# OpenDriveLab/OccNet

Measured on NVIDIA H100. Metric: samples/s (6-cam->200x200x16 voxel), higher is better.
Workload: dtype bf16

## Files before the change

### include/occ_b200.h

```cpp
#ifndef OCC_B200_H_
#define OCC_B200_H_

#include <stdint.h>

#ifdef __cplusplus
extern "C" {
#endif

const char* occb200_last_error(void);
const char* occb200_version(void);

int occb200_ms_deform_attn_forward(const float* value, const int64_t* spatial_shapes,
                                   const int64_t* level_start_index, const float* sampling_loc,
                                   const float* attn_weight, int B, int Nv, int M, int C, int Nq, int L, int P,
                                   int im2col_step, float* out, void* stream);

int occb200_ms_deform_attn_backward(const float* value, const int64_t* spatial_shapes, const int64_t* level_start_index,
                                    const float* sampling_loc, const float* attn_weight, const float* grad_output, int B,
                                    int Nv, int M, int C, int Nq, int L, int P, int im2col_step, float* grad_value,
                                    float* grad_sampling_loc, float* grad_attn_weight, void* stream);

typedef struct occb200_engine occb200_engine;
typedef struct occb200_backbone occb200_backbone;

typedef struct occb200_config {
    int bev_h, bev_w;
    int embed_dims, num_heads;
    int num_layers;
    int num_cams;
    int num_levels;
    int level_h[4], level_w[4];
    int num_points_in_pillar;
    int sca_points, tsa_points;
    int ffn_dim;
    int pillar_h, out_dim;
    int num_classes;
    float pc_range[6];
    int precision;
    int use_tensor_cores;
    int use_cams_embeds;
    int rotate_center[2];
} occb200_config;

int occb200_engine_create(const occb200_config* cfg, occb200_engine** out);
void occb200_engine_destroy(occb200_engine* e);

int occb200_engine_load_param(occb200_engine* e, const char* key, const float* data, int64_t numel);
int occb200_engine_finalize(occb200_engine* e);

int occb200_engine_set_cameras(occb200_engine* e, const float* cam_mat, const float* zs, int img_h, int img_w);

int occb200_engine_set_prev_rotation(occb200_engine* e, const int32_t* map_host);

int occb200_engine_set_input_dtype(occb200_engine* e, int feats_bf16);
int occb200_engine_attach_backbone(occb200_engine* e, occb200_backbone* bb);

int occb200_engine_forward(occb200_engine* e, const float* const* feats, const float* prev_bev, float* bev_embed,
                           float* occ_logits, float* flow, uint8_t* occ_cls_u8, int64_t* occ_cls_i64, void* stream);

int occb200_engine_forward_host(occb200_engine* e, const float* const* feats_host, int64_t* occ_cls_i64_host,
                                float* flow_host, void* stream);

int occb200_engine_submit_host(occb200_engine* e, int slot, const float* const* feats_host, int64_t* occ_cls_i64_host,
                               float* flow_host, void* stream);
int occb200_engine_wait_host(occb200_engine* e, int slot);

int occb200_engine_enable_taps(occb200_engine* e, int enable);
int occb200_engine_copy_tap(occb200_engine* e, int which, int layer, float* dst_dev, void* stream);

int occb200_engine_project_pillars(occb200_engine* e, float* ref_cam, uint8_t* mask, void* stream);
int occb200_engine_launches_per_frame(const occb200_engine* e);
int occb200_engine_profile(occb200_engine* e, int enable);
int occb200_engine_profile_read(occb200_engine* e, float* ms_per_category, int* launches_per_category, int n);

int occb200_render_forward(const float* sigma, const float* origin, const float* points, const float* tindex,
                           int N, int T, int Z, int Y, int X, int64_t M, float* pred_dist, float* gt_dist,
                           float* coord_index, void* stream);

int occb200_ray_metric_accumulate(const uint8_t* sem_pred, const float* flow_pred, const uint8_t* sem_gt,
                                  const float* flow_gt, const void* origins, int origin_is_f64, int T,
                                  const float* rays, int M, double* counters, float* pcd_pred, float* pcd_gt,
                                  void* stream);

int occb200_linear_f32(const float* A, const float* W, const float* bias, const float* residual, float* C, int M,
                       int N, int K, int act, void* stream);
int occb200_layernorm_f32(const float* x, const float* gamma, const float* beta, float* y, int rows, int C,
                          void* stream);
int occb200_gemm_bf16_tc(const void* A_bf16, const void* W_bf16, const float* bias, float* C, int M, int N, int K,
                         void* stream);

occb200_backbone* occb200_backbone_create(int num_images, int img_h, int img_w, int precision, int use_tensor_cores);
void occb200_backbone_destroy(occb200_backbone* e);
int occb200_backbone_load_param(occb200_backbone* e, const char* key, const float* data, int64_t numel);
int occb200_backbone_finalize(occb200_backbone* e);
int occb200_backbone_level_shape(const occb200_backbone* e, int level, int* h, int* w);
int occb200_backbone_forward(occb200_backbone* e, const float* img, float* out0, float* out1, float* out2, float* out3,
                             void* stream);
int occb200_backbone_forward_nhwc_bf16(occb200_backbone* e, const float* img, void* out0, void* out1, void* out2, void* out3,
                                       void* stream);
int occb200_backbone_set_frame_format(occb200_backbone* e, int src_h, int src_w, const float mean[3], const float std[3],
                                      int to_rgb);
int occb200_backbone_forward_frames(occb200_backbone* e, const uint8_t* frames, void* out0, void* out1, void* out2,
                                    void* out3, int out_layout, void* stream);

#ifdef __cplusplus
}
#endif
#endif
```

### occnet_b200/_lib.py

```python
import ctypes
import os

_HERE = os.path.dirname(os.path.abspath(__file__))
LIB_PATH = os.path.join(_HERE, 'lib', 'libocc_b200.so')

c_f32p = ctypes.c_void_p
_vp = ctypes.c_void_p
_i = ctypes.c_int
_i64 = ctypes.c_int64


class OccConfig(ctypes.Structure):
    _fields_ = [('bev_h', _i), ('bev_w', _i), ('embed_dims', _i), ('num_heads', _i), ('num_layers', _i),
                ('num_cams', _i), ('num_levels', _i), ('level_h', _i * 4), ('level_w', _i * 4),
                ('num_points_in_pillar', _i), ('sca_points', _i), ('tsa_points', _i), ('ffn_dim', _i),
                ('pillar_h', _i), ('out_dim', _i), ('num_classes', _i), ('pc_range', ctypes.c_float * 6),
                ('precision', _i), ('use_tensor_cores', _i), ('use_cams_embeds', _i),
                ('rotate_center', _i * 2)]


SIGNATURES = {
    'occb200_last_error': (ctypes.c_char_p, []),
    'occb200_version': (ctypes.c_char_p, []),
    'occb200_ms_deform_attn_forward': (_i, [_vp, _vp, _vp, _vp, _vp, _i, _i, _i, _i, _i, _i, _i, _i, _vp, _vp]),
    'occb200_ms_deform_attn_backward': (_i, [_vp, _vp, _vp, _vp, _vp, _vp, _i, _i, _i, _i, _i, _i, _i, _i, _vp, _vp, _vp, _vp]),
    'occb200_engine_create': (_i, [ctypes.POINTER(OccConfig), ctypes.POINTER(_vp)]),
    'occb200_engine_destroy': (None, [_vp]),
    'occb200_engine_load_param': (_i, [_vp, ctypes.c_char_p, _vp, _i64]),
    'occb200_engine_finalize': (_i, [_vp]),
    'occb200_engine_set_cameras': (_i, [_vp, _vp, _vp, _i, _i]),
    'occb200_engine_set_input_dtype': (_i, [_vp, _i]),
    'occb200_engine_attach_backbone': (_i, [_vp, _vp]),
    'occb200_engine_set_prev_rotation': (_i, [_vp, _vp]),
    'occb200_engine_forward': (_i, [_vp, ctypes.POINTER(_vp), _vp, _vp, _vp, _vp, _vp, _vp, _vp]),
    'occb200_engine_forward_host': (_i, [_vp, ctypes.POINTER(_vp), _vp, _vp, _vp]),
    'occb200_engine_submit_host': (_i, [_vp, _i, ctypes.POINTER(_vp), _vp, _vp, _vp]),
    'occb200_engine_wait_host': (_i, [_vp, _i]),
    'occb200_engine_enable_taps': (_i, [_vp, _i]),
    'occb200_engine_copy_tap': (_i, [_vp, _i, _i, _vp, _vp]),
    'occb200_engine_project_pillars': (_i, [_vp, _vp, _vp, _vp]),
    'occb200_engine_launches_per_frame': (_i, [_vp]),
    'occb200_engine_profile': (_i, [_vp, _i]),
    'occb200_engine_profile_read': (_i, [_vp, _vp, _vp, _i]),
    'occb200_render_forward': (_i, [_vp, _vp, _vp, _vp, _i, _i, _i, _i, _i, _i64, _vp, _vp, _vp, _vp]),
    'occb200_ray_metric_accumulate': (_i, [_vp, _vp, _vp, _vp, _vp, _i, _i, _vp, _i, _vp, _vp, _vp, _vp]),
    'occb200_linear_f32': (_i, [_vp, _vp, _vp, _vp, _vp, _i, _i, _i, _i, _vp]),
    'occb200_layernorm_f32': (_i, [_vp, _vp, _vp, _vp, _i, _i, _vp]),
    'occb200_gemm_bf16_tc': (_i, [_vp, _vp, _vp, _vp, _i, _i, _i, _vp]),
    'occb200_backbone_create': (_vp, [_i, _i, _i, _i, _i]),
    'occb200_backbone_destroy': (None, [_vp]),
    'occb200_backbone_load_param': (_i, [_vp, ctypes.c_char_p, _vp, ctypes.c_int64]),
    'occb200_backbone_finalize': (_i, [_vp]),
    'occb200_backbone_level_shape': (_i, [_vp, _i, ctypes.POINTER(_i), ctypes.POINTER(_i)]),
    'occb200_backbone_forward': (_i, [_vp, _vp, _vp, _vp, _vp, _vp, _vp]),
    'occb200_backbone_forward_nhwc_bf16': (_i, [_vp, _vp, _vp, _vp, _vp, _vp, _vp]),
    'occb200_backbone_set_frame_format': (_i, [_vp, _i, _i, _vp, _vp, _i]),
    'occb200_backbone_forward_frames': (_i, [_vp, _vp, _vp, _vp, _vp, _vp, _i, _vp]),
}

_lib = None


def load():
    global _lib
    if _lib is None:
        if not os.path.exists(LIB_PATH):
            raise RuntimeError(f'{LIB_PATH} is missing: run `python -m occnet_b200.build` '
                               '(libocc_b200 has no CPU / PyTorch fallback)')
        lib = ctypes.CDLL(LIB_PATH)
        for name, (res, args) in SIGNATURES.items():
            fn = getattr(lib, name)
            fn.restype = res
            fn.argtypes = args
        _lib = lib
    return _lib


class OccB200Error(RuntimeError):
    pass


def check(rc):
    if rc != 0:
        raise OccB200Error(f'libocc_b200 error {rc}: {load().occb200_last_error().decode()}')


def ptr(t):
    if t is None:
        return None
    if hasattr(t, 'data_ptr'):
        return ctypes.c_void_p(t.data_ptr())
    return ctypes.c_void_p(t.ctypes.data)


def stream_ptr():
    import torch
    return ctypes.c_void_p(torch.cuda.current_stream().cuda_stream)
```

### occnet_b200/csrc/engine.cu

```cuda
#include <cuda_runtime.h>

#include <algorithm>
#include <cmath>
#include <cstring>
#include <map>
#include <string>
#include <vector>

#include "../../include/occ_b200.h"
#include "common.cuh"
#include "conv3d_tc.cuh"
#include "gemm_tc.cuh"
#include "kernels.cuh"

namespace occ {

static thread_local std::string g_last_error;
void set_last_error(const std::string& msg) { g_last_error = msg; }

namespace {

struct DevBuf {
    void* p = nullptr;
    size_t bytes = 0;
// ... 1075 lines not shown
    OCC_CHECK(e && (slot == 0 || slot == 1), "bad arguments");
    occb200_engine::Slot& s = e->slots[slot];
    if (!s.busy) return 0;
    OCC_CUDA(cudaEventSynchronize(s.d2h_done));
    s.busy = false;
    return 0;
}

int occb200_engine_set_prev_rotation(occb200_engine* e, const int32_t* map_host)
{
    OCC_CHECK(e, "null engine");
    if (map_host == nullptr) { e->rot_set = false; return 0; }
    for (int q = 0; q < e->Nq; ++q) OCC_CHECK(map_host[q] >= -1 && map_host[q] < e->Nq, "rotation map entry out of range");
    if (e->rot_map.bytes != (size_t)e->Nq * 4 && e->rot_map.alloc((size_t)e->Nq * 4)) return 2;
    OCC_CUDA(cudaMemcpy(e->rot_map.p, map_host, (size_t)e->Nq * 4, cudaMemcpyHostToDevice));
    e->rot_set = true;
    return 0;
}

int occb200_engine_set_input_dtype(occb200_engine* e, int feats_bf16)
{
    OCC_CHECK(e && feats_bf16 >= 0 && feats_bf16 <= 3,
              "input dtype must be 0 (fp32 NCHW), 1 (bf16 NCHW), 2 (bf16 NHWC) or 3 (uint8 camera frames)");
    e->feats_bf16 = feats_bf16;
    return 0;
}

int occb200_engine_attach_backbone(occb200_engine* e, occb200_backbone* bb)
{
    OCC_CHECK(e, "null engine");
    if (bb && check_backbone(e, bb)) return 1;
    if (e->bb_free_recorded) OCC_CUDA(cudaEventSynchronize(e->bb_free));
    e->bb = bb;
    e->bb_free_recorded = false;
    return 0;
}

int occb200_engine_enable_taps(occb200_engine* e, int enable)
{
    OCC_CHECK(e && e->finalized, "engine not finalized");
    e->taps = enable != 0;
    if (e->taps) {
        const size_t n = (size_t)e->cfg.num_layers * e->Nq * 256 * 4;
        if (e->tap_layer.alloc(n) || e->tap_tsa.alloc(n) || e->tap_sca.alloc(n)) return 2;
    }
    return 0;
}

int occb200_engine_copy_tap(occb200_engine* e, int which, int layer, float* dst, void* stream)
{
    OCC_CHECK(e && dst, "null pointer");
    cudaStream_t st = (cudaStream_t)stream;
    const size_t n = (size_t)e->Nq * 256;
    if (which >= 0 && which <= 2) {
        OCC_CHECK(e->taps && layer >= 0 && layer < e->cfg.num_layers, "taps not enabled or bad layer");
        const DevBuf& b = which == 0 ? e->tap_layer : (which == 1 ? e->tap_tsa : e->tap_sca);
        OCC_CUDA(cudaMemcpyAsync(dst, b.as<float>() + layer * n, n * 4, cudaMemcpyDeviceToDevice, st));
        return 0;
    }
    if (which == 3) {
        const size_t nv = (size_t)e->cfg.bev_w * e->cfg.bev_h * e->cfg.pillar_h * e->cfg.out_dim;
        if (e->cfg.precision == 0) {
            OCC_CUDA(cudaMemcpyAsync(dst, e->vox2.p, nv * 4, cudaMemcpyDeviceToDevice, st));
            return 0;
        }
        return launch_bf16_to_f32(e->vox2.as<bf16>(), dst, (int64_t)nv, st);
    }
    if (which == 4) {
        const size_t nt = (size_t)e->cfg.num_cams * e->Nv * 256;
        if (e->cfg.precision == 0) {
            OCC_CUDA(cudaMemcpyAsync(dst, e->tokens.p, nt * 4, cudaMemcpyDeviceToDevice, st));
            return 0;
        }
        return launch_bf16_to_f32(e->tokens.as<bf16>(), dst, (int64_t)nt, st);
    }
    set_last_error("unknown tap");
    return 1;
}

int occb200_engine_project_pillars(occb200_engine* e, float* ref_cam, uint8_t* mask, void* stream)
{
    OCC_CHECK(e && ref_cam && mask && e->cameras_set, "null pointer / cameras not set");
    return launch_project_pillars(e->sp, ref_cam, mask, (cudaStream_t)stream);
}

int occb200_engine_launches_per_frame(const occb200_engine* e) { return e ? e->launches : 0; }

int occb200_engine_profile(occb200_engine* e, int enable)
{
    OCC_CHECK(e, "null engine");
    e->profiling = enable != 0;
    e->prof_events.clear();
    e->event_used = 0;
    return 0;
}

int occb200_engine_profile_read(occb200_engine* e, float* ms_per_category, int* launches_per_category, int n)
{
    OCC_CHECK(e && ms_per_category && launches_per_category && n >= CAT_COUNT, "bad arguments");
    OCC_CUDA(cudaDeviceSynchronize());
    for (int i = 0; i < n; ++i) { ms_per_category[i] = 0.f; launches_per_category[i] = 0; }
    for (auto& pe : e->prof_events) {
        float ms = 0.f;
        OCC_CUDA(cudaEventElapsedTime(&ms, pe.second.first, pe.second.second));
        ms_per_category[pe.first] += ms;
        launches_per_category[pe.first] += 1;
    }
    e->prof_events.clear();
    e->event_used = 0;
    return 0;
}

int occb200_render_forward(const float* sigma, const float* origin, const float* points, const float* tindex, int N,
                           int T, int Z, int Y, int X, int64_t M, float* pred_dist, float* gt_dist, float* coord_index,
                           void* stream)
{
    OCC_CHECK(sigma && origin && points && tindex && pred_dist && gt_dist && coord_index, "null pointer");
    return launch_render_forward(sigma, origin, points, tindex, N, T, Z, Y, X, M, pred_dist, gt_dist, coord_index,
                                 (cudaStream_t)stream);
}

int occb200_ray_metric_accumulate(const uint8_t* sem_pred, const float* flow_pred, const uint8_t* sem_gt,
                                  const float* flow_gt, const void* origins, int origin_is_f64, int T, const float* rays,
                                  int M, double* counters, float* pcd_pred, float* pcd_gt, void* stream)
{
    if (T == 0 || M == 0) return 0;
    OCC_CHECK(sem_pred && flow_pred && sem_gt && flow_gt && origins && rays && counters, "null pointer");
    return launch_ray_metric(sem_pred, flow_pred, sem_gt, flow_gt, origins, origin_is_f64, T, rays, M, counters,
                             pcd_pred, pcd_gt, (cudaStream_t)stream);
}

int occb200_linear_f32(const float* A, const float* W, const float* bias, const float* residual, float* C, int M, int N,
                       int K, int act, void* stream)
{
    OCC_CHECK(A && W && C, "null pointer");
    return gemm_simt<float, float>(A, K, nullptr, 0, K, W, bias, residual, N, C, N, M, N, K, act, (cudaStream_t)stream);
}

int occb200_layernorm_f32(const float* x, const float* gamma, const float* beta, float* y, int rows, int C, void* stream)
{
    OCC_CHECK(x && gamma && beta && y, "null pointer");
    return launch_layernorm<float>(x, gamma, beta, nullptr, rows, C, y, (float*)nullptr, (float*)nullptr,
                                   (cudaStream_t)stream);
}

int occb200_gemm_bf16_tc(const void* A, const void* W, const float* bias, float* C, int M, int N, int K, void* stream)
{
    OCC_CHECK(A && W && C, "null pointer");
    OCC_CHECK(gemm_tc_supported(M, N, K, K), "shape not supported by the tensor-core GEMM");
    return gemm_tc<float>(reinterpret_cast<const bf16*>(A), nullptr, 0, reinterpret_cast<const bf16*>(W), bias, nullptr,
                          C, M, N, K, ACT_NONE, (cudaStream_t)stream);
}

}
```

### occnet_b200/csrc/gemm_tc.cu

```cuda
#include <cstdlib>
#include <map>
#include <mutex>
#include <tuple>
#include <type_traits>

#include "gemm_tc.cuh"
#include "tc_common.cuh"

namespace occ {

PFN_encodeTiled get_encode_tiled()
{
    static PFN_encodeTiled fn = nullptr;
    static std::once_flag once;
    std::call_once(once, [] {
        void* p = nullptr;
        cudaDriverEntryPointQueryResult q;
        if (cudaGetDriverEntryPoint("cuTensorMapEncodeTiled", &p, cudaEnableDefault, &q) == cudaSuccess &&
            q == cudaDriverEntryPointSuccess)
            fn = reinterpret_cast<PFN_encodeTiled>(p);
    });
    return fn;
}

int make_tensor_map_bf16(CUtensorMap* map, const void* base, int rank, const uint64_t* dims, const uint64_t* strides_bytes,
                         const uint32_t* box, int swizzle_bytes)
{
    PFN_encodeTiled enc = get_encode_tiled();
    OCC_CHECK(enc != nullptr, "cuTensorMapEncodeTiled is not available from the driver");
    cuuint64_t gdim[5], gstr[5];
    cuuint32_t bdim[5], estr[5];
    for (int i = 0; i < rank; ++i) { gdim[i] = dims[i]; bdim[i] = box[i]; estr[i] = 1; }
    for (int i = 0; i + 1 < rank; ++i) gstr[i] = strides_bytes[i];
    const CUtensorMapSwizzle sw = swizzle_bytes == 128 ? CU_TENSOR_MAP_SWIZZLE_128B
                                : swizzle_bytes == 64 ? CU_TENSOR_MAP_SWIZZLE_64B
                                : swizzle_bytes == 32 ? CU_TENSOR_MAP_SWIZZLE_32B : CU_TENSOR_MAP_SWIZZLE_NONE;
    const CUresult r = enc(map, CU_TENSOR_MAP_DATA_TYPE_BFLOAT16, (cuuint32_t)rank, const_cast<void*>(base), gdim, gstr,
                           bdim, estr, CU_TENSOR_MAP_INTERLEAVE_NONE, sw, CU_TENSOR_MAP_L2_PROMOTION_L2_128B,
                           CU_TENSOR_MAP_FLOAT_OOB_FILL_NONE);
    OCC_CHECK(r == CUDA_SUCCESS, "cuTensorMapEncodeTiled failed with code " + std::to_string((int)r));
    return 0;
}

int cached_map_2d(const void* base, uint64_t inner, uint64_t rows, uint32_t box_inner, uint32_t box_rows, CUtensorMap* out,
                  uint64_t ld = 0);

namespace {

constexpr int BLOCK_M = 128, BLOCK_K = 64, A_TILE_BYTES = BLOCK_M * BLOCK_K * 2;
constexpr int NUM_THREADS = 384;
constexpr int SMEM_TAIL = 3072 + 256;
constexpr int SMEM_MAX = 232448 - 1024;
constexpr int MAX_STAGES = 6;

struct LnArgs {
    const float* gamma; const float* beta; const float* pos;
    float* y_f32; bf16* y_bf16; bf16* y_pos_bf16;
};

constexpr int MAX_PROBS = 3;
struct GemmProb {
    CUtensorMap tmA, tmA2, tmW;
    const float* bias; const float* residual; void* C;
    const float* res_t32;
    long long ldc, nblk_stride;
    int head_major;
    int M, N, BN, nk, nk1, act, w_resident, stages;
    int out_half;
    int cta_begin, cta_count;
};
struct GemmProbs { GemmProb p[MAX_PROBS]; int n; };

template <typename TC, bool LN>
__global__ void __launch_bounds__(NUM_THREADS, 1)
gemm_tc_kernel(const __grid_constant__ GemmProbs probs, LnArgs ln)
{
    int pi = 0;
    while (pi + 1 < probs.n && (int)blockIdx.x >= probs.p[pi + 1].cta_begin) ++pi;
    const GemmProb& P = probs.p[pi];
    const float* __restrict__ residual = P.residual;
    const float* __restrict__ res_t32 = P.res_t32;
    const int M = P.M, N = P.N, BN = P.BN, nk = P.nk, nk1 = P.nk1, act = P.act;
    const int w_resident = P.w_resident, stages = P.stages;
    const bool out_half = std::is_same<TC, __half>::value || P.out_half != 0;
    const int bid = (int)blockIdx.x - P.cta_begin, nctas = P.cta_count;
    asm volatile("griddepcontrol.launch_dependents;" ::: "memory");
    extern __shared__ uint8_t smem_raw[];
    const uint32_t smem_base = (tc::smem_u32(smem_raw) + 1023u) & ~1023u;
    const uint32_t w_tile_bytes = BN * BLOCK_K * 2;
    const uint32_t w_region = w_resident ? nk * w_tile_bytes : 0;
    const uint32_t stage_bytes = A_TILE_BYTES + (w_resident ? 0 : w_tile_bytes);
    const uint32_t ring_base = smem_base + w_region;
    const uint32_t cvec_base = ring_base + stages * stage_bytes;
    const uint32_t bar_base = cvec_base + 3072;
    auto full_bar = [&](int s) { return bar_base + s * 8; };
    auto empty_bar = [&](int s) { return bar_base + (MAX_STAGES + s) * 8; };
    auto w_bar = [&](int kb) { return bar_base + (2 * MAX_STAGES + (kb < 7 ? kb : 7)) * 8; };
    float* const cvec = reinterpret_cast<float*>(smem_raw + (cvec_base - tc::smem_u32(smem_raw)));

    const int warp = threadIdx.x >> 5, lane = threadIdx.x & 31;
    const int n_tiles = N / BN;
    const int n_blk = bid % n_tiles;
    const int grp = bid / n_tiles, ngrp = nctas / n_tiles;
    const int nb32 = (M + 31) >> 5;
    const int row_begin = (int)(((long long)nb32 * grp) / ngrp) << 5;
    const int row_end = min(M, (int)(((long long)nb32 * (grp + 1)) / ngrp) << 5);

    if (warp == 8 && lane == 0) {
        tc::tma_prefetch_desc(&P.tmA); tc::tma_prefetch_desc(&P.tmA2); tc::tma_prefetch_desc(&P.tmW);
        for (int s = 0; s < stages; ++s) { tc::mbar_init(full_bar(s), 1); tc::mbar_init(empty_bar(s), 2); }
        for (int kb = 0; kb < 8; ++kb) tc::mbar_init(w_bar(kb), 1);
        tc::mbar_fence_init();
    }
    if (threadIdx.x < BN) {
        const int t = threadIdx.x;
        cvec[t] = P.bias ? __ldg(P.bias + n_blk * BN + t) : 0.f;
        if constexpr (LN) { cvec[256 + t] = __ldg(ln.gamma + t); cvec[512 + t] = __ldg(ln.beta + t); }
    }
    __syncthreads();

    if (warp >= 8) {
        tc::setmaxnreg_dec<40>();
        if (warp == 8 && lane == 0) {
            if (w_resident) {
                for (int kb = 0; kb < nk && kb < 8; ++kb)
                    tc::mbar_arrive_expect_tx(w_bar(kb), kb < 7 ? w_tile_bytes : (nk - 7) * w_tile_bytes);
                for (int kb = 0; kb < nk; ++kb)
                    tc::tma_load_2d(smem_base + kb * w_tile_bytes, &P.tmW, w_bar(kb), kb * BLOCK_K, n_blk * BN);
            }
            int s = 0; uint32_t ph = 0;
            asm volatile("griddepcontrol.wait;" ::: "memory");
            for (int m_row = row_begin; m_row < row_end; m_row += BLOCK_M) {
                for (int kb = 0; kb < nk; ++kb) {
                    tc::mbar_wait(empty_bar(s), ph ^ 1);
                    tc::mbar_arrive_expect_tx(full_bar(s), stage_bytes);
                    const uint32_t a_dst = ring_base + s * stage_bytes;
                    if (kb < nk1) tc::tma_load_2d(a_dst, &P.tmA, full_bar(s), kb * BLOCK_K, m_row);
                    else          tc::tma_load_2d(a_dst, &P.tmA2, full_bar(s), (kb - nk1) * BLOCK_K, m_row);
                    if (!w_resident)
                        tc::tma_load_2d(a_dst + A_TILE_BYTES, &P.tmW, full_bar(s), kb * BLOCK_K, n_blk * BN);
                    if (++s == stages) { s = 0; ph ^= 1; }
                }
            }
        }
        return;
    }

    tc::setmaxnreg_inc<232>();
    const int wg = warp >> 2, wl = warp & 3;
    const int nsubs = BN >> 6;
    const int quad_col = 2 * (lane & 3);
    int s = 0; uint32_t ph = 0;
    int tcount = 0;
    asm volatile("griddepcontrol.wait;" ::: "memory");
    for (int m_row = row_begin; m_row < row_end; m_row += BLOCK_M, ++tcount) {
        float acc[4][32];
        for (int kb = 0; kb < nk; ++kb) {
            if (w_resident && tcount == 0) tc::mbar_wait(w_bar(kb), 0);
            tc::mbar_wait(full_bar(s), ph);
            const uint32_t a_addr = ring_base + s * stage_bytes + wg * (64 * 128);
            const uint32_t b_addr = w_resident ? smem_base + kb * w_tile_bytes : ring_base + s * stage_bytes + A_TILE_BYTES;
            switch (nsubs) {
            case 4: tc::wgmma_kblock<4>(acc, a_addr, b_addr, kb == 0); break;
            case 3: tc::wgmma_kblock<3>(acc, a_addr, b_addr, kb == 0); break;
            case 2: tc::wgmma_kblock<2>(acc, a_addr, b_addr, kb == 0); break;
            default: tc::wgmma_kblock<1>(acc, a_addr, b_addr, kb == 0); break;
            }
            if ((threadIdx.x & 127) == 0) tc::mbar_arrive(empty_bar(s));
            if (++s == stages) { s = 0; ph ^= 1; }
        }
        const int r0 = m_row + wg * 64 + wl * 16 + (lane >> 2);
        if constexpr (LN) {
            tc::ln_epilogue(acc, r0, row_end, quad_col, cvec, residual, ln.pos, ln.y_f32, ln.y_bf16, ln.y_pos_bf16);
        } else {
            const bool has_t32 = res_t32 != nullptr, has_res = residual != nullptr, relu = act == ACT_RELU;
            const float* __restrict__ qsrc = has_t32 ? res_t32 : residual;
            const int q_blk = has_t32 ? 1024 : 32, q_j = has_t32 ? 256 : 8;
            const size_t o_blk = P.head_major ? (size_t)M * 32 : 32;
#pragma unroll
            for (int h = 0; h < 2; ++h) {
                const int row = r0 + 8 * h;
                if (row >= row_end) continue;
                const float* const qrow =
                    qsrc + (has_t32 ? ((((size_t)(row >> 5) * (N >> 5) + n_blk * (BN >> 5)) * 256 + (quad_col >> 2) * 32 + (row & 31)) << 2) +
                                          (quad_col & 3)
                                    : (size_t)row * N + n_blk * BN + quad_col);
                float2 q[4][8];
                if (qsrc) {
#pragma unroll
                    for (int ns = 0; ns < 4; ++ns) {
                        if (ns >= nsubs) break;
#pragma unroll
                        for (int j = 0; j < 8; ++j)
                            q[ns][j] = __ldg(reinterpret_cast<const float2*>(qrow + (2 * ns + j / 4) * q_blk + (j & 3) * q_j));
                    }
                }
                TC* const orow = reinterpret_cast<TC*>(P.C) +
                                 (P.head_major ? ((size_t)n_blk * (BN >> 5) * M + row) * 32 + quad_col
                                               : (size_t)n_blk * P.nblk_stride + (size_t)row * P.ldc + quad_col);
#pragma unroll
                for (int ns = 0; ns < 4; ++ns) {
                    if (ns >= nsubs) break;
#pragma unroll
                    for (int j = 0; j < 8; ++j) {
                        const int cl = ns * 64 + 8 * j + quad_col;
                        float x0 = acc[ns][4 * j + 2 * h] + cvec[cl], x1 = acc[ns][4 * j + 2 * h + 1] + cvec[cl + 1];
                        if (has_t32) { x0 += q[ns][j].x; x1 += q[ns][j].y; }
                        if (relu) { x0 = fmaxf(x0, 0.f); x1 = fmaxf(x1, 0.f); }
                        if (has_res) { x0 += q[ns][j].x; x1 += q[ns][j].y; }
                        TC* const o = orow + (2 * ns + j / 4) * o_blk + 8 * (j & 3);
                        if constexpr (sizeof(TC) == 4)
                            *reinterpret_cast<float2*>(o) = make_float2(x0, x1);
                        else
                            *reinterpret_cast<uint32_t*>(o) = tc::pack_16(x0, x1, out_half);
                    }
                }
            }
        }
    }
}

struct Plan { int BN, resident, stages, smem; };

Plan make_plan(int N, int K, bool ln)
{
    const int SMEM_LIMIT = SMEM_MAX - SMEM_TAIL;
    Plan p{0, 0, 0, 0};
    const int cands[] = {256, 192, 128, 64};
    if (ln) {
        p.BN = 256;
    } else {
        for (int bn : cands) {
            if (N % bn != 0 || bn > N) continue;
            if ((long)bn * K * 2 <= 131072) { p.BN = bn; break; }
        }
        if (K > 512 && p.BN != 0 && p.BN < 128) p.BN = 0;
        if (p.BN == 0) {
            for (int bn : cands) if (N % bn == 0 && bn <= N) { p.BN = bn; break; }
        }
    }
    if (p.BN == 0) return p;
    const int w_bytes = p.BN * K * 2;
    p.resident = w_bytes <= 131072;
    const int stage = A_TILE_BYTES + (p.resident ? 0 : p.BN * BLOCK_K * 2);
    const int avail = SMEM_LIMIT - (p.resident ? w_bytes : 0);
    p.stages = avail / stage;
    if (p.stages > MAX_STAGES) p.stages = MAX_STAGES;
    p.smem = 1024 + (p.resident ? w_bytes : 0) + p.stages * stage + SMEM_TAIL;
    return p;
}

struct MapKey {
    const void* p; uint64_t d0, d1, ld; uint32_t b0, b1;
    bool operator<(const MapKey& o) const { return std::tie(p, d0, d1, ld, b0, b1) < std::tie(o.p, o.d0, o.d1, o.ld, o.b0, o.b1); }
};

}

int cached_map_2d(const void* base, uint64_t inner, uint64_t rows, uint32_t box_inner, uint32_t box_rows, CUtensorMap* out,
                  uint64_t ld)
{
    static std::map<MapKey, CUtensorMap> cache;
    static std::mutex mu;
    std::lock_guard<std::mutex> g(mu);
    if (ld == 0) ld = inner;
    const MapKey k{base, inner, rows, ld, box_inner, box_rows};
    auto it = cache.find(k);
    if (it == cache.end()) {
        CUtensorMap m;
        const uint64_t dims[2] = {inner, rows}, strides[1] = {ld * 2};
        const uint32_t box[2] = {box_inner, box_rows};
        if (make_tensor_map_bf16(&m, base, 2, dims, strides, box, 128)) return 1;
        if (cache.size() > 4096) cache.clear();
        it = cache.emplace(k, m).first;
    }
    *out = it->second;
    return 0;
}

namespace {

template <typename TC, bool LN>
int build_prob(GemmProb& P, int& smem, const bf16* A, const bf16* A2, int K1, const bf16* W, const float* bias, const float* residual,
               TC* C, int M, int N, int K, int act, bool blocked_out, int lda, int lda2, bool head_major, int ctas, int cta_begin)
{
    if (A2 == nullptr) K1 = K;
    const Plan p = make_plan(N, K, LN);
    OCC_CHECK(p.BN > 0 && p.stages >= 2 && K % 64 == 0 && K1 % 64 == 0 && M > 0, "gemm_tc: unsupported shape");
    if (cached_map_2d(A, (uint64_t)K1, (uint64_t)M, BLOCK_K, BLOCK_M, &P.tmA, (uint64_t)lda)) return 1;
    if (A2) { if (cached_map_2d(A2, (uint64_t)(K - K1), (uint64_t)M, BLOCK_K, BLOCK_M, &P.tmA2, (uint64_t)lda2)) return 1; }
    else P.tmA2 = P.tmA;
    if (cached_map_2d(W, (uint64_t)K, (uint64_t)N, BLOCK_K, (uint32_t)p.BN, &P.tmW)) return 1;
    if (ctas <= 0) ctas = sm_count_current_device();
    const int m_tiles = (M + BLOCK_M - 1) / BLOCK_M, n_tiles = N / p.BN;
    int per_n = ctas / n_tiles;
    if (per_n > m_tiles) per_n = m_tiles;
    OCC_CHECK(per_n >= 1, "gemm_tc: fewer CTAs than n-blocks");
    P.bias = bias; P.residual = residual; P.C = C; P.res_t32 = nullptr;
    P.ldc = blocked_out ? (long long)p.BN : (long long)N;
    P.nblk_stride = blocked_out ? (long long)M * p.BN : (long long)p.BN;
    P.head_major = head_major ? 1 : 0;
    P.M = M; P.N = N; P.BN = p.BN; P.nk = K / BLOCK_K; P.nk1 = K1 / BLOCK_K; P.act = act;
    P.w_resident = p.resident; P.stages = p.stages;
    P.out_half = std::is_same<TC, __half>::value ? 1 : 0;
    P.cta_begin = cta_begin; P.cta_count = per_n * n_tiles;
    smem = p.smem;
    return 0;
}

template <typename TC, bool LN>
int launch_probs(const GemmProbs& probs, int smem, LnArgs ln, cudaStream_t stream)
{
    OCC_CUDA(cudaFuncSetAttribute(gemm_tc_kernel<TC, LN>, cudaFuncAttributeMaxDynamicSharedMemorySize, 232448));
    const GemmProb& last = probs.p[probs.n - 1];
    const int grid = last.cta_begin + last.cta_count;
    cudaLaunchConfig_t cfg = {};
    cfg.gridDim = dim3(grid); cfg.blockDim = dim3(NUM_THREADS); cfg.dynamicSmemBytes = smem; cfg.stream = stream;
    cudaLaunchAttribute attr[1];
    attr[0].id = cudaLaunchAttributeProgrammaticStreamSerialization;
    attr[0].val.programmaticStreamSerializationAllowed = 1;
    cfg.attrs = attr; cfg.numAttrs = 1;
    OCC_CUDA(cudaLaunchKernelEx(&cfg, gemm_tc_kernel<TC, LN>, probs, ln));
    OCC_CUDA(cudaGetLastError());
    return 0;
}

template <typename TC, bool LN>
int launch(const bf16* A, const bf16* A2, int K1, const bf16* W, const float* bias, const float* residual, TC* C,
           LnArgs ln, int M, int N, int K, int act, cudaStream_t stream, bool blocked_out = false, int lda = 0, int lda2 = 0,
           bool head_major = false)
{
    GemmProbs probs;
    probs.n = 1;
    int smem = 0;
    if (build_prob<TC, LN>(probs.p[0], smem, A, A2, K1, W, bias, residual, C, M, N, K, act, blocked_out, lda, lda2, head_major, 0, 0))
        return 1;
    return launch_probs<TC, LN>(probs, smem, ln, stream);
}

}

bool gemm_tc_supported(int M, int N, int K, int K1)
{
    const Plan p = make_plan(N, K, false);
    return M > 0 && p.BN >= 64 && p.BN % 64 == 0 && p.stages >= 2 && K % 64 == 0 && K1 % 64 == 0 && K1 > 0 && K1 <= K;
}

template <typename TC>
int gemm_tc(const bf16* A, const bf16* A2, int K1, const bf16* W, const float* bias, const float* residual, TC* C,
            int M, int N, int K, int act, cudaStream_t stream)
{
    return launch<TC, false>(A, A2, K1, W, bias, residual, C, LnArgs{}, M, N, K, act, stream);
}

int gemm_tc_heads256(const bf16* A, const bf16* W, const float* bias, bf16* C, int M, int K, cudaStream_t stream)
{
    return launch<bf16, false>(A, nullptr, 0, W, bias, nullptr, C, LnArgs{}, M, 256, K, ACT_NONE, stream, false, 0, 0, true);
}

int gemm_tc_split3(const bf16* S, int Ks, const bf16* W3, const float* bias, const float* residual, float* C, int M, int N,
                   int act, cudaStream_t stream)
{
    return launch<float, false>(S, S, 2 * Ks, W3, bias, residual, C, LnArgs{}, M, N, 3 * Ks, act, stream, false, 2 * Ks, 2 * Ks);
}

int gemm_tc_blocked256(const bf16* A, const bf16* W, const float* bias, bf16* C, int M, int N, int K, cudaStream_t stream,
                       bool head_major)
{
    const Plan p = make_plan(N, K, false);
    OCC_CHECK(p.BN == 256 && N % 256 == 0, "gemm_tc_blocked256: N must be a multiple of 256 with 256-wide tiles");
    return launch<bf16, false>(A, nullptr, 0, W, bias, nullptr, C, LnArgs{}, M, N, K, ACT_NONE, stream, true, 0, 0, head_major);
}

int gemm_tc_ln(const bf16* A, const bf16* W, const float* bias, const float* residual, const float* gamma,
               const float* beta, const float* pos, float* y_f32, bf16* y_bf16, bf16* y_pos_bf16, int M, int K,
               cudaStream_t stream)
{
    OCC_CHECK(bias && residual && gamma && beta, "gemm_tc_ln: bias, residual, gamma, beta are required");
    OCC_CHECK(y_pos_bf16 == nullptr || pos != nullptr, "gemm_tc_ln: pos required for y_pos");
    return launch<float, true>(A, nullptr, 0, W, bias, residual, (float*)nullptr, LnArgs{gamma, beta, pos, y_f32, y_bf16, y_pos_bf16},
                               M, 256, K, ACT_NONE, stream);
}

int gemm_tc_tsa_inputs(const bf16* const* Av, int nv, const bf16* Wv, const float* bv, bf16* const* Cv, const bf16* Aq,
                       const bf16* Aq2, int K1q, const bf16* Wq, const float* bq, const float* rq, const float* rq_t32, __half* Cq,
                       int M, int Nq, int Kq, cudaStream_t stream)
{
    OCC_CHECK(nv >= 1 && nv <= 2, "gemm_tc_tsa_inputs: 1 or 2 value problems");
    const int num_sms = sm_count_current_device();
    const double wv = 256.0 * 256.0, wq = (double)Nq * Kq, tot = nv * wv + wq;
    int cq = (int)(num_sms * wq / tot + 0.5);
    const int nq_tiles = Nq / make_plan(Nq, Kq, false).BN;
    if (cq < nq_tiles) cq = nq_tiles;
    const int cv = (num_sms - cq) / nv;
    OCC_CHECK(cv >= 1, "gemm_tc_tsa_inputs: not enough SMs");
    GemmProbs probs;
    probs.n = nv + 1;
    int smem = 0, sm = 0, begin = 0;
    for (int i = 0; i < nv; ++i) {
        if (build_prob<bf16, false>(probs.p[i], sm, Av[i], nullptr, 0, Wv, bv, nullptr, Cv[i], M, 256, 256, ACT_NONE, false, 0, 0,
                                    false, cv, begin)) return 1;
        begin += probs.p[i].cta_count;
        smem = sm > smem ? sm : smem;
    }
    const bool t32 = rq_t32 != nullptr && M % 32 == 0;
    if (build_prob<bf16, false>(probs.p[nv], sm, Aq, Aq2, K1q, Wq, bq, t32 ? nullptr : rq, reinterpret_cast<bf16*>(Cq), M, Nq, Kq,
                                ACT_NONE, false, 0, 0, false, cq, begin)) return 1;
    probs.p[nv].out_half = 1;
    if (t32) probs.p[nv].res_t32 = rq_t32;
    smem = sm > smem ? sm : smem;
    return launch_probs<bf16, false>(probs, smem, LnArgs{}, stream);
}

template int gemm_tc<float>(const bf16*, const bf16*, int, const bf16*, const float*, const float*, float*, int, int,
                            int, int, cudaStream_t);
template int gemm_tc<bf16>(const bf16*, const bf16*, int, const bf16*, const float*, const float*, bf16*, int, int, int,
                           int, cudaStream_t);
template int gemm_tc<__half>(const bf16*, const bf16*, int, const bf16*, const float*, const float*, __half*, int, int, int,
                             int, cudaStream_t);

}
```

### occnet_b200/csrc/tc_common.cuh

```cuda
#pragma once
#include <cuda.h>
#include <cuda_runtime.h>
#include <stdint.h>

#include "common.cuh"

namespace occ {
namespace tc {

__device__ __forceinline__ uint32_t smem_u32(const void* p) { return (uint32_t)__cvta_generic_to_shared(p); }

__device__ __forceinline__ void mbar_init(uint32_t bar, uint32_t count)
{
    asm volatile("mbarrier.init.shared::cta.b64 [%0], %1;" ::"r"(bar), "r"(count) : "memory");
}
__device__ __forceinline__ void mbar_fence_init()
{
    asm volatile("fence.mbarrier_init.release.cluster;" ::: "memory");
    asm volatile("fence.proxy.async.shared::cta;" ::: "memory");
}
__device__ __forceinline__ void mbar_arrive_expect_tx(uint32_t bar, uint32_t bytes)
{
    asm volatile("mbarrier.arrive.expect_tx.shared::cta.b64 _, [%0], %1;" ::"r"(bar), "r"(bytes) : "memory");
}
__device__ __forceinline__ void mbar_arrive(uint32_t bar)
{
    asm volatile("mbarrier.arrive.shared::cta.b64 _, [%0];" ::"r"(bar) : "memory");
}
__device__ __forceinline__ bool mbar_try_wait(uint32_t bar, uint32_t parity)
{
    uint32_t ok;
    asm volatile(
        "{\n\t.reg .pred p;\n\t"
        "mbarrier.try_wait.parity.shared::cta.b64 p, [%1], %2;\n\t"
        "selp.u32 %0, 1, 0, p;\n\t}"
        : "=r"(ok)
        : "r"(bar), "r"(parity)
        : "memory");
    return ok != 0;
}
__device__ __forceinline__ void mbar_wait(uint32_t bar, uint32_t parity)
{
    uint32_t spins = 0;
    while (!mbar_try_wait(bar, parity)) {
        if (++spins > 20000000u) { asm volatile("trap;"); }
    }
}

__device__ __forceinline__ void tma_prefetch_desc(const void* desc)
{
    asm volatile("prefetch.tensormap [%0];" ::"l"(desc) : "memory");
}
__device__ __forceinline__ void tma_load_2d(uint32_t dst, const void* desc, uint32_t bar, int c0, int c1)
{
    asm volatile(
        "cp.async.bulk.tensor.2d.shared::cluster.global.mbarrier::complete_tx::bytes [%0], [%1, {%3, %4}], [%2];"
        ::"r"(dst), "l"(desc), "r"(bar), "r"(c0), "r"(c1)
        : "memory");
}
__device__ __forceinline__ void tma_load_4d(uint32_t dst, const void* desc, uint32_t bar, int c0, int c1, int c2, int c3)
{
    asm volatile(
        "cp.async.bulk.tensor.4d.shared::cluster.global.mbarrier::complete_tx::bytes [%0], [%1, {%3, %4, %5, %6}], [%2];"
        ::"r"(dst), "l"(desc), "r"(bar), "r"(c0), "r"(c1), "r"(c2), "r"(c3)
        : "memory");
}

template <int N> __device__ __forceinline__ void setmaxnreg_inc() { asm volatile("setmaxnreg.inc.sync.aligned.u32 %0;" ::"n"(N)); }
template <int N> __device__ __forceinline__ void setmaxnreg_dec() { asm volatile("setmaxnreg.dec.sync.aligned.u32 %0;" ::"n"(N)); }
__device__ __forceinline__ void wgmma_fence() { asm volatile("wgmma.fence.sync.aligned;" ::: "memory"); }
__device__ __forceinline__ void wgmma_commit() { asm volatile("wgmma.commit_group.sync.aligned;" ::: "memory"); }
__device__ __forceinline__ void wgmma_wait_all() { asm volatile("wgmma.wait_group.sync.aligned 0;" ::: "memory"); }
template <int R>
__device__ __forceinline__ void reg_fence(float (&d)[R])
{
#pragma unroll
    for (int i = 0; i < R; ++i) asm volatile("" : "+f"(d[i])::"memory");
}
#define OCC_ACC8(i) "+f"(d[i]), "+f"(d[i + 1]), "+f"(d[i + 2]), "+f"(d[i + 3]), "+f"(d[i + 4]), "+f"(d[i + 5]), "+f"(d[i + 6]), "+f"(d[i + 7])
__device__ __forceinline__ void wgmma_m64n32(float (&d)[16], uint64_t desc_a, uint64_t desc_b, uint32_t accumulate)
{
    asm volatile(
        "{\n\t.reg .pred p;\n\t"
        "setp.ne.b32 p, %18, 0;\n\t"
        "wgmma.mma_async.sync.aligned.m64n32k16.f32.bf16.bf16 "
        "{%0, %1, %2, %3, %4, %5, %6, %7, %8, %9, %10, %11, %12, %13, %14, %15}, %16, %17, p, 1, 1, 0, 0;\n\t}"
        : OCC_ACC8(0), OCC_ACC8(8)
        : "l"(desc_a), "l"(desc_b), "r"(accumulate)
        : "memory");
}
__device__ __forceinline__ void wgmma_m64n64(float (&d)[32], uint64_t desc_a, uint64_t desc_b, uint32_t accumulate)
{
    asm volatile(
        "{\n\t.reg .pred p;\n\t"
        "setp.ne.b32 p, %34, 0;\n\t"
        "wgmma.mma_async.sync.aligned.m64n64k16.f32.bf16.bf16 "
        "{%0, %1, %2, %3, %4, %5, %6, %7, %8, %9, %10, %11, %12, %13, %14, %15, %16, %17, %18, %19, %20, %21, %22, %23, %24, %25, %26, %27, %28, %29, %30, %31}, %32, %33, p, 1, 1, 0, 0;\n\t}"
        : OCC_ACC8(0), OCC_ACC8(8), OCC_ACC8(16), OCC_ACC8(24)
        : "l"(desc_a), "l"(desc_b), "r"(accumulate)
        : "memory");
}
__device__ __forceinline__ void wgmma_m64n96(float (&d)[48], uint64_t desc_a, uint64_t desc_b, uint32_t accumulate)
{
    asm volatile(
        "{\n\t.reg .pred p;\n\t"
        "setp.ne.b32 p, %50, 0;\n\t"
        "wgmma.mma_async.sync.aligned.m64n96k16.f32.bf16.bf16 "
        "{%0, %1, %2, %3, %4, %5, %6, %7, %8, %9, %10, %11, %12, %13, %14, %15, %16, %17, %18, %19, %20, %21, %22, %23, %24, %25, %26, %27, %28, %29, %30, %31, %32, %33, %34, %35, %36, %37, %38, %39, %40, %41, %42, %43, %44, %45, %46, %47}, %48, %49, p, 1, 1, 0, 0;\n\t}"
        : OCC_ACC8(0), OCC_ACC8(8), OCC_ACC8(16), OCC_ACC8(24), OCC_ACC8(32), OCC_ACC8(40)
        : "l"(desc_a), "l"(desc_b), "r"(accumulate)
        : "memory");
}
__device__ __forceinline__ void wgmma_m64n128(float (&d)[64], uint64_t desc_a, uint64_t desc_b, uint32_t accumulate)
{
    asm volatile(
        "{\n\t.reg .pred p;\n\t"
        "setp.ne.b32 p, %66, 0;\n\t"
        "wgmma.mma_async.sync.aligned.m64n128k16.f32.bf16.bf16 "
        "{%0, %1, %2, %3, %4, %5, %6, %7, %8, %9, %10, %11, %12, %13, %14, %15, %16, %17, %18, %19, %20, %21, %22, %23, %24, %25, %26, %27, %28, %29, %30, %31, %32, %33, %34, %35, %36, %37, %38, %39, %40, %41, %42, %43, %44, %45, %46, %47, %48, %49, %50, %51, %52, %53, %54, %55, %56, %57, %58, %59, %60, %61, %62, %63}, %64, %65, p, 1, 1, 0, 0;\n\t}"
        : OCC_ACC8(0), OCC_ACC8(8), OCC_ACC8(16), OCC_ACC8(24), OCC_ACC8(32), OCC_ACC8(40), OCC_ACC8(48), OCC_ACC8(56)
        : "l"(desc_a), "l"(desc_b), "r"(accumulate)
        : "memory");
}

__device__ __forceinline__ uint64_t make_smem_desc(uint32_t smem_addr, uint32_t row_bytes)
{
    const uint64_t layout = row_bytes == 128 ? 1 : (row_bytes == 64 ? 2 : 3);
    uint64_t d = 0;
    d |= (uint64_t)((smem_addr & 0x3FFFF) >> 4);
    d |= (uint64_t)1 << 16;
    d |= (uint64_t)((8 * row_bytes) >> 4) << 32;
    d |= layout << 62;
    return d;
}

__device__ __forceinline__ size_t t32_index(int row, int col, int ncols)
{
    return ((((size_t)(row >> 5) * (ncols >> 5) + (col >> 5)) * 256 + ((col & 31) >> 2) * 32 + (row & 31)) << 2) + (col & 3);
}

__device__ __forceinline__ uint32_t pack_16(float a, float b, bool half)
{
    if (half) {
        const __half2 h = __floats2half2_rn(a, b);
        return *reinterpret_cast<const uint32_t*>(&h);
    }
    return pack_bf16x2(a, b);
}

__device__ __forceinline__ void ln_epilogue(float (&acc)[4][32], int r0, int row_end, int quad_col, const float* cvec,
                                            const float* residual, const float* pos, float* y_f32, bf16* y_bf16, bf16* y_pos_bf16)
{
    auto ld2 = [](const float* p) {
        float2 v;
        asm volatile("ld.global.v2.f32 {%0, %1}, [%2];" : "=f"(v.x), "=f"(v.y) : "l"(p) : "memory");
        return v;
    };
    float mean[2], rstd[2];
#pragma unroll
    for (int h = 0; h < 2; ++h) {
        const int row = r0 + 8 * h;
        float sum = 0.f, sumsq = 0.f;
#pragma unroll
        for (int ns = 0; ns < 4; ++ns) {
#pragma unroll
            for (int j = 0; j < 8; ++j) {
                const int c = ns * 64 + 8 * j + quad_col;
                const float2 q = row < row_end ? ld2(residual + t32_index(row, c, 256)) : make_float2(0.f, 0.f);
                const float x0 = acc[ns][4 * j + 2 * h] + cvec[c] + q.x, x1 = acc[ns][4 * j + 2 * h + 1] + cvec[c + 1] + q.y;
                acc[ns][4 * j + 2 * h] = x0; acc[ns][4 * j + 2 * h + 1] = x1;
                sum += x0 + x1;
                sumsq = fmaf(x0, x0, fmaf(x1, x1, sumsq));
            }
        }
        sum += __shfl_xor_sync(0xffffffffu, sum, 1); sum += __shfl_xor_sync(0xffffffffu, sum, 2);
        sumsq += __shfl_xor_sync(0xffffffffu, sumsq, 1); sumsq += __shfl_xor_sync(0xffffffffu, sumsq, 2);
        mean[h] = sum * (1.f / 256.f);
        const float var = fmaxf(sumsq * (1.f / 256.f) - mean[h] * mean[h], 0.f);
        rstd[h] = rsqrtf(var + 1e-5f);
    }
#pragma unroll
    for (int h = 0; h < 2; ++h) {
        const int row = r0 + 8 * h;
        if (row >= row_end) continue;
#pragma unroll
        for (int ns = 0; ns < 4; ++ns) {
#pragma unroll
            for (int j = 0; j < 8; ++j) {
                const int c = ns * 64 + 8 * j + quad_col;
                const float y0 = (acc[ns][4 * j + 2 * h] - mean[h]) * rstd[h] * cvec[256 + c] + cvec[512 + c];
                const float y1 = (acc[ns][4 * j + 2 * h + 1] - mean[h]) * rstd[h] * cvec[256 + c + 1] + cvec[512 + c + 1];
                const size_t ti = t32_index(row, c, 256);
                if (y_f32) *reinterpret_cast<float2*>(y_f32 + ti) = make_float2(y0, y1);
                if (y_bf16) *reinterpret_cast<uint32_t*>(y_bf16 + (size_t)row * 256 + c) = pack_bf16x2(y0, y1);
                if (y_pos_bf16) {
                    const float2 p = __ldg(reinterpret_cast<const float2*>(pos + ti));
                    *reinterpret_cast<uint32_t*>(y_pos_bf16 + (size_t)row * 256 + c) = pack_bf16x2(y0 + p.x, y1 + p.y);
                }
            }
        }
    }
}

template <int NS>
__device__ __forceinline__ void wgmma_kblock(float (&acc)[4][32], uint32_t a_addr, uint32_t b_addr, bool first)
{
    const uint64_t da = make_smem_desc(a_addr, 128);
    wgmma_fence();
#pragma unroll
    for (int k = 0; k < 4; ++k) {
#pragma unroll
        for (int ns = 0; ns < NS; ++ns)
            wgmma_m64n64(acc[ns], da + 2 * k, make_smem_desc(b_addr + ns * (64 * 128), 128) + 2 * k, !(first && k == 0));
    }
    wgmma_commit();
    wgmma_wait_all();
#pragma unroll
    for (int ns = 0; ns < NS; ++ns) reg_fence(acc[ns]);
}

}

inline int sm_count_current_device()
{
    static int cache[64] = {0};
    int dev = 0;
    if (cudaGetDevice(&dev) != cudaSuccess || dev < 0 || dev >= 64) return 132;
    if (cache[dev] == 0) cudaDeviceGetAttribute(&cache[dev], cudaDevAttrMultiProcessorCount, dev);
    return cache[dev] > 0 ? cache[dev] : 132;
}

typedef CUresult (*PFN_encodeTiled)(CUtensorMap*, CUtensorMapDataType, cuuint32_t, void*, const cuuint64_t*,
                                    const cuuint64_t*, const cuuint32_t*, const cuuint32_t*, CUtensorMapInterleave,
                                    CUtensorMapSwizzle, CUtensorMapL2promotion, CUtensorMapFloatOOBfill);
PFN_encodeTiled get_encode_tiled();
int make_tensor_map_bf16(CUtensorMap* map, const void* base, int rank, const uint64_t* dims, const uint64_t* strides_bytes,
                         const uint32_t* box, int swizzle_bytes);

}
```

Baseline: 169.1.

## Ping-pong consumer warpgroups over 64-row tiles with async wgmma overlap

The GEMM consumer is restructured so the two math warpgroups alternate over independent 64-row M tiles, ping-pong style, instead of splitting one 128-row tile. Named barriers order the handoff between the warpgroups so one can run its epilogue while the other issues MMAs. Within a tile, wgmma groups are now kept in flight one k-block deep, and a stage is released only after the previous group retires. Stage count and barrier arrival counts are adjusted to match, and a new C entry point exposes the GEMM variants for testing. This adds barrier coordination complexity and halves the A tile per stage.

```diff
diff --git a/include/occ_b200.h b/include/occ_b200.h
--- a/include/occ_b200.h
+++ b/include/occ_b200.h
@@ -88,6 +88,10 @@
                           void* stream);
 int occb200_gemm_bf16_tc(const void* A_bf16, const void* W_bf16, const float* bias, float* C, int M, int N, int K,
                          void* stream);
+int occb200_gemm_tc_variant(int kind, const void* A, const void* W, const float* bias, const float* residual, void* C, int M,
+                            int N, int K, int act, int out_dtype, int head_major, const void* A2, const void* W2,
+                            const float* bias2, const float* res_t32, void* C2, int N2, int K2, const float* gamma,
+                            const float* beta, const float* pos, float* y_f32, void* y_bf16, void* y_pos_bf16, void* stream);
 
 occb200_backbone* occb200_backbone_create(int num_images, int img_h, int img_w, int precision, int use_tensor_cores);
 void occb200_backbone_destroy(occb200_backbone* e);
diff --git a/occnet_b200/_lib.py b/occnet_b200/_lib.py
--- a/occnet_b200/_lib.py
+++ b/occnet_b200/_lib.py
@@ -47,6 +47,8 @@
     'occb200_linear_f32': (_i, [_vp, _vp, _vp, _vp, _vp, _i, _i, _i, _i, _vp]),
     'occb200_layernorm_f32': (_i, [_vp, _vp, _vp, _vp, _i, _i, _vp]),
     'occb200_gemm_bf16_tc': (_i, [_vp, _vp, _vp, _vp, _i, _i, _i, _vp]),
+    'occb200_gemm_tc_variant': (_i, [_i, _vp, _vp, _vp, _vp, _vp, _i, _i, _i, _i, _i, _i, _vp, _vp, _vp, _vp, _vp, _i, _i,
+                                     _vp, _vp, _vp, _vp, _vp, _vp, _vp]),
     'occb200_backbone_create': (_vp, [_i, _i, _i, _i, _i]),
     'occb200_backbone_destroy': (None, [_vp]),
     'occb200_backbone_load_param': (_i, [_vp, ctypes.c_char_p, _vp, ctypes.c_int64]),
diff --git a/occnet_b200/csrc/engine.cu b/occnet_b200/csrc/engine.cu
--- a/occnet_b200/csrc/engine.cu
+++ b/occnet_b200/csrc/engine.cu
@@ -1251,4 +1251,39 @@
                           C, M, N, K, ACT_NONE, (cudaStream_t)stream);
 }
 
-}
+int occb200_gemm_tc_variant(int kind, const void* A, const void* W, const float* bias, const float* residual, void* C, int M,
+                            int N, int K, int act, int out_dtype, int head_major, const void* A2, const void* W2,
+                            const float* bias2, const float* res_t32, void* C2, int N2, int K2, const float* gamma,
+                            const float* beta, const float* pos, float* y_f32, void* y_bf16, void* y_pos_bf16, void* stream)
+{
+    OCC_CHECK(A && W, "null pointer");
+    const bf16* a = reinterpret_cast<const bf16*>(A);
+    const bf16* w = reinterpret_cast<const bf16*>(W);
+    const cudaStream_t s = (cudaStream_t)stream;
+    switch (kind) {
+    case 0:
+        OCC_CHECK(C && gemm_tc_supported(M, N, K, K) && act >= 0 && act <= 1, "unsupported plain GEMM");
+        if (out_dtype == 0) return gemm_tc<float>(a, nullptr, 0, w, bias, residual, (float*)C, M, N, K, act, s);
+        if (out_dtype == 1) return gemm_tc<bf16>(a, nullptr, 0, w, bias, residual, (bf16*)C, M, N, K, act, s);
+        if (out_dtype == 2) return gemm_tc<__half>(a, nullptr, 0, w, bias, residual, (__half*)C, M, N, K, act, s);
+        OCC_CHECK(false, "out_dtype must be 0 (fp32), 1 (bf16) or 2 (fp16)");
+    case 1:
+        OCC_CHECK(C, "null pointer");
+        if (head_major && N == 256) return gemm_tc_heads256(a, w, bias, (bf16*)C, M, K, s);
+        return gemm_tc_blocked256(a, w, bias, (bf16*)C, M, N, K, s, head_major != 0);
+    case 2:
+        OCC_CHECK(N == 256 && residual && gamma && beta, "LayerNorm GEMM: N = 256, residual, gamma, beta required");
+        return gemm_tc_ln(a, w, bias, residual, gamma, beta, pos, y_f32, (bf16*)y_bf16, (bf16*)y_pos_bf16, M, K, s);
+    case 3: {
+        OCC_CHECK(C && A2 && W2 && C2 && N == 256 && K == 256, "TSA inputs: value GEMM N = K = 256, projection operands required");
+        bf16* cv = (bf16*)C;
+        return gemm_tc_tsa_inputs(&a, 1, w, bias, &cv, reinterpret_cast<const bf16*>(A2), nullptr, K2,
+                                  reinterpret_cast<const bf16*>(W2), bias2, nullptr, res_t32, (__half*)C2, M, N2, K2, s);
+    }
+    default:
+        OCC_CHECK(false, "kind must be 0..3");
+    }
+    return 1;
+}
+
+}
diff --git a/occnet_b200/csrc/gemm_tc.cu b/occnet_b200/csrc/gemm_tc.cu
--- a/occnet_b200/csrc/gemm_tc.cu
+++ b/occnet_b200/csrc/gemm_tc.cu
@@ -47,11 +47,12 @@
 
 namespace {
 
-constexpr int BLOCK_M = 128, BLOCK_K = 64, A_TILE_BYTES = BLOCK_M * BLOCK_K * 2;
+constexpr int TILE_M = 64, BLOCK_K = 64, A_TILE_BYTES = TILE_M * BLOCK_K * 2;
 constexpr int NUM_THREADS = 384;
 constexpr int SMEM_TAIL = 3072 + 256;
 constexpr int SMEM_MAX = 232448 - 1024;
-constexpr int MAX_STAGES = 6;
+constexpr int MAX_STAGES = 12;
+constexpr int BAR_TURN = 2;
 
 struct LnArgs {
     const float* gamma; const float* beta; const float* pos;
@@ -108,7 +109,7 @@
 
     if (warp == 8 && lane == 0) {
         tc::tma_prefetch_desc(&P.tmA); tc::tma_prefetch_desc(&P.tmA2); tc::tma_prefetch_desc(&P.tmW);
-        for (int s = 0; s < stages; ++s) { tc::mbar_init(full_bar(s), 1); tc::mbar_init(empty_bar(s), 2); }
+        for (int s = 0; s < stages; ++s) { tc::mbar_init(full_bar(s), 1); tc::mbar_init(empty_bar(s), 1); }
         for (int kb = 0; kb < 8; ++kb) tc::mbar_init(w_bar(kb), 1);
         tc::mbar_fence_init();
     }
@@ -130,7 +131,7 @@
             }
             int s = 0; uint32_t ph = 0;
             asm volatile("griddepcontrol.wait;" ::: "memory");
-            for (int m_row = row_begin; m_row < row_end; m_row += BLOCK_M) {
+            for (int m_row = row_begin; m_row < row_end; m_row += TILE_M) {
                 for (int kb = 0; kb < nk; ++kb) {
                     tc::mbar_wait(empty_bar(s), ph ^ 1);
                     tc::mbar_arrive_expect_tx(full_bar(s), stage_bytes);
@@ -150,26 +151,42 @@
     const int wg = warp >> 2, wl = warp & 3;
     const int nsubs = BN >> 6;
     const int quad_col = 2 * (lane & 3);
+    const bool elected = (threadIdx.x & 127) == 0;
+    const int ntiles = (row_end - row_begin + TILE_M - 1) / TILE_M;
     int s = 0; uint32_t ph = 0;
-    int tcount = 0;
+    auto skip = [&](int n) { for (int i = 0; i < n; ++i) if (++s == stages) { s = 0; ph ^= 1; } };
+    if (wg == 1) skip(nk);
     asm volatile("griddepcontrol.wait;" ::: "memory");
-    for (int m_row = row_begin; m_row < row_end; m_row += BLOCK_M, ++tcount) {
+    for (int t = wg; t < ntiles; t += 2) {
+        const int m_row = row_begin + t * TILE_M;
+        if (t > 0) tc::named_bar_sync(BAR_TURN + wg, 256);
         float acc[4][32];
+        int s_prev = 0;
         for (int kb = 0; kb < nk; ++kb) {
-            if (w_resident && tcount == 0) tc::mbar_wait(w_bar(kb), 0);
+            if (w_resident && t < 2) tc::mbar_wait(w_bar(kb), 0);
             tc::mbar_wait(full_bar(s), ph);
-            const uint32_t a_addr = ring_base + s * stage_bytes + wg * (64 * 128);
+            const uint32_t a_addr = ring_base + s * stage_bytes;
             const uint32_t b_addr = w_resident ? smem_base + kb * w_tile_bytes : ring_base + s * stage_bytes + A_TILE_BYTES;
             switch (nsubs) {
-            case 4: tc::wgmma_kblock<4>(acc, a_addr, b_addr, kb == 0); break;
-            case 3: tc::wgmma_kblock<3>(acc, a_addr, b_addr, kb == 0); break;
-            case 2: tc::wgmma_kblock<2>(acc, a_addr, b_addr, kb == 0); break;
-            default: tc::wgmma_kblock<1>(acc, a_addr, b_addr, kb == 0); break;
+            case 4: tc::wgmma_kblock_issue<4>(acc, a_addr, b_addr, kb == 0); break;
+            case 3: tc::wgmma_kblock_issue<3>(acc, a_addr, b_addr, kb == 0); break;
+            case 2: tc::wgmma_kblock_issue<2>(acc, a_addr, b_addr, kb == 0); break;
+            default: tc::wgmma_kblock_issue<1>(acc, a_addr, b_addr, kb == 0); break;
             }
-            if ((threadIdx.x & 127) == 0) tc::mbar_arrive(empty_bar(s));
+            if (kb > 0) {
+                tc::wgmma_wait_1();
+                if (elected) tc::mbar_arrive(empty_bar(s_prev));
+            }
+            s_prev = s;
             if (++s == stages) { s = 0; ph ^= 1; }
         }
-        const int r0 = m_row + wg * 64 + wl * 16 + (lane >> 2);
+        tc::wgmma_wait_all();
+#pragma unroll
+        for (int ns = 0; ns < 4; ++ns) tc::reg_fence(acc[ns]);
+        if (elected) tc::mbar_arrive(empty_bar(s_prev));
+        if (t + 1 < ntiles) tc::named_bar_arrive(BAR_TURN + (wg ^ 1), 256);
+        skip(nk);
+        const int r0 = m_row + wl * 16 + (lane >> 2);
         if constexpr (LN) {
             tc::ln_epilogue(acc, r0, row_end, quad_col, cvec, residual, ln.pos, ln.y_f32, ln.y_bf16, ln.y_pos_bf16);
         } else {
@@ -287,12 +304,12 @@
     if (A2 == nullptr) K1 = K;
     const Plan p = make_plan(N, K, LN);
     OCC_CHECK(p.BN > 0 && p.stages >= 2 && K % 64 == 0 && K1 % 64 == 0 && M > 0, "gemm_tc: unsupported shape");
-    if (cached_map_2d(A, (uint64_t)K1, (uint64_t)M, BLOCK_K, BLOCK_M, &P.tmA, (uint64_t)lda)) return 1;
-    if (A2) { if (cached_map_2d(A2, (uint64_t)(K - K1), (uint64_t)M, BLOCK_K, BLOCK_M, &P.tmA2, (uint64_t)lda2)) return 1; }
+    if (cached_map_2d(A, (uint64_t)K1, (uint64_t)M, BLOCK_K, TILE_M, &P.tmA, (uint64_t)lda)) return 1;
+    if (A2) { if (cached_map_2d(A2, (uint64_t)(K - K1), (uint64_t)M, BLOCK_K, TILE_M, &P.tmA2, (uint64_t)lda2)) return 1; }
     else P.tmA2 = P.tmA;
     if (cached_map_2d(W, (uint64_t)K, (uint64_t)N, BLOCK_K, (uint32_t)p.BN, &P.tmW)) return 1;
     if (ctas <= 0) ctas = sm_count_current_device();
-    const int m_tiles = (M + BLOCK_M - 1) / BLOCK_M, n_tiles = N / p.BN;
+    const int m_tiles = (M + 2 * TILE_M - 1) / (2 * TILE_M), n_tiles = N / p.BN;
     int per_n = ctas / n_tiles;
     if (per_n > m_tiles) per_n = m_tiles;
     OCC_CHECK(per_n >= 1, "gemm_tc: fewer CTAs than n-blocks");
diff --git a/occnet_b200/csrc/tc_common.cuh b/occnet_b200/csrc/tc_common.cuh
--- a/occnet_b200/csrc/tc_common.cuh
+++ b/occnet_b200/csrc/tc_common.cuh
@@ -64,6 +64,15 @@
         "cp.async.bulk.tensor.4d.shared::cluster.global.mbarrier::complete_tx::bytes [%0], [%1, {%3, %4, %5, %6}], [%2];"
         ::"r"(dst), "l"(desc), "r"(bar), "r"(c0), "r"(c1), "r"(c2), "r"(c3)
         : "memory");
+}
+
+__device__ __forceinline__ void named_bar_sync(int id, int threads)
+{
+    asm volatile("bar.sync %0, %1;" ::"r"(id), "r"(threads) : "memory");
+}
+__device__ __forceinline__ void named_bar_arrive(int id, int threads)
+{
+    asm volatile("bar.arrive %0, %1;" ::"r"(id), "r"(threads) : "memory");
 }
 
 template <int N> __device__ __forceinline__ void setmaxnreg_inc() { asm volatile("setmaxnreg.inc.sync.aligned.u32 %0;" ::"n"(N)); }
@@ -71,6 +80,7 @@
 __device__ __forceinline__ void wgmma_fence() { asm volatile("wgmma.fence.sync.aligned;" ::: "memory"); }
 __device__ __forceinline__ void wgmma_commit() { asm volatile("wgmma.commit_group.sync.aligned;" ::: "memory"); }
 __device__ __forceinline__ void wgmma_wait_all() { asm volatile("wgmma.wait_group.sync.aligned 0;" ::: "memory"); }
+__device__ __forceinline__ void wgmma_wait_1() { asm volatile("wgmma.wait_group.sync.aligned 1;" ::: "memory"); }
 template <int R>
 __device__ __forceinline__ void reg_fence(float (&d)[R])
 {
@@ -203,7 +213,7 @@
 }
 
 template <int NS>
-__device__ __forceinline__ void wgmma_kblock(float (&acc)[4][32], uint32_t a_addr, uint32_t b_addr, bool first)
+__device__ __forceinline__ void wgmma_kblock_issue(float (&acc)[4][32], uint32_t a_addr, uint32_t b_addr, bool first)
 {
     const uint64_t da = make_smem_desc(a_addr, 128);
     wgmma_fence();
@@ -214,6 +224,11 @@
             wgmma_m64n64(acc[ns], da + 2 * k, make_smem_desc(b_addr + ns * (64 * 128), 128) + 2 * k, !(first && k == 0));
     }
     wgmma_commit();
+}
+template <int NS>
+__device__ __forceinline__ void wgmma_kblock(float (&acc)[4][32], uint32_t a_addr, uint32_t b_addr, bool first)
+{
+    wgmma_kblock_issue<NS>(acc, a_addr, b_addr, first);
     wgmma_wait_all();
 #pragma unroll
     for (int ns = 0; ns < NS; ++ns) reg_fence(acc[ns]);
```

Result: faster. 172.2 (median of 6 runs) (+1.8%).
